# KTH-RPL/cloth-splatting

Hardware: AMD Instinct MI355X
Metric: rasterizer fwd+bwd rendered Mpix/s (scene_1, 800x800) (higher is better)
Workload: dtype f32

## Files before the change

cloth-splatting_amd/csrc/csplat_raster.hip:

```cpp
#include "csplat_common.h"

#include <atomic>
#include <cstring>
#include <chrono>
#include <mutex>
#include <type_traits>

namespace {

constexpr float NEAR_Z = 0.2f;
constexpr int RASTER_MAX_VIEWS = 8;

__device__ constexpr float SH_C0 = 0.28209479177387814f;
__device__ constexpr float SH_C1 = 0.4886025119029199f;
__device__ constexpr float SH_C2[5] = {1.0925484305920792f, -1.0925484305920792f, 0.31539156525252005f,
                                       -1.0925484305920792f, 0.5462742152960396f};
__device__ constexpr float SH_C3[7] = {-0.5900435899266435f, 2.890611442640554f, -0.4570457994644658f,
                                       0.3731763325901154f, -0.4570457994644658f, 1.445305721320277f,
                                       -0.5900435899266435f};

struct Geom {
    float *depth;
    float2 *xy;
    float4 *conic_opacity;
// ... 406 lines not shown
    extern __shared__ uint32_t s_hist[];
    for (int t = threadIdx.x; t < tiles; t += BUCKET_G) s_hist[t] = 0u;
    __syncthreads();
    const int i = blockIdx.x * BUCKET_G + threadIdx.x;
    if (i < P) {
        const int rad = radii[i];
        if (rad > 0) {
            const float2 p = xy[i];
            int minx, miny, maxx, maxy;
            tile_rect(p.x, p.y, rad, cam, minx, miny, maxx, maxy);
            for (int y = miny; y < maxy; y++)
                for (int x = minx; x < maxx; x++) atomicAdd(&s_hist[y * cam.gx + x], 1u);
        }
    }
    __syncthreads();
    uint32_t *row = table + (size_t)blockIdx.x * tiles;
    for (int t = threadIdx.x; t < tiles; t += BUCKET_G) row[t] = s_hist[t];
}
__global__ __launch_bounds__(BUCKET_G) void k_tile_count(int P, int tiles, const float2 *__restrict__ xy,
                                                          const int32_t *__restrict__ radii, Cam cam,
                                                          uint32_t *__restrict__ table) {
    tile_count_body(P, tiles, xy, radii, cam, table);
}
__global__ __launch_bounds__(BUCKET_G) void k_tile_count_views(int P, int tiles, K1Table tab) {
    const K1View &w = tab.v[blockIdx.y];
    tile_count_body(P, tiles, w.g.xy, w.radii, w.cam, w.table);
}

__device__ __forceinline__ void tile_colscan_body(int tiles, int nb, uint32_t *__restrict__ table, uint32_t *__restrict__ cnt) {
    const int t = blockIdx.x * 256 + threadIdx.x;
    if (t >= tiles) return;
    uint32_t run = 0;
    int b = 0;
    for (; b + 8 <= nb; b += 8) {
        uint32_t v[8];
#pragma unroll
        for (int u = 0; u < 8; u++) v[u] = table[(size_t)(b + u) * tiles + t];
#pragma unroll
        for (int u = 0; u < 8; u++) { table[(size_t)(b + u) * tiles + t] = run; run += v[u]; }
    }
    for (; b < nb; b++) { const uint32_t v = table[(size_t)b * tiles + t]; table[(size_t)b * tiles + t] = run; run += v; }
    cnt[t] = run;
}
__global__ __launch_bounds__(256) void k_tile_colscan(int tiles, int nb, uint32_t *__restrict__ table, uint32_t *__restrict__ cnt) {
    tile_colscan_body(tiles, nb, table, cnt);
}
__global__ __launch_bounds__(256) void k_tile_colscan_views(int tiles, int nb, K1Table tab) {
    uint32_t *table = tab.v[blockIdx.y].table;
    tile_colscan_body(tiles, nb, table, table + (size_t)nb * tiles);
}

constexpr int INFO_BUSY = 64;
constexpr int LPT_BINS = 512;
__device__ __forceinline__ void tile_scan_body(int tiles, const uint32_t *__restrict__ cnt, int2 *__restrict__ ranges,
                                               uint32_t *__restrict__ info, volatile uint32_t *mailbox, uint32_t tag) {
    __shared__ unsigned long long s_w[17];
    __shared__ uint32_t s_max[16];
    const int lane = threadIdx.x & 63, w = threadIdx.x >> 6;
    unsigned long long carry = 0ull;
    uint32_t mx = 0;
    uint32_t *busy = info + INFO_BUSY;
    for (int base = 0; base < tiles; base += 1024) {
        const int t = base + threadIdx.x;
        const uint32_t c = t < tiles ? cnt[t] : 0u;
        mx = max(mx, c);
        const unsigned long long v0 = (unsigned long long)c | ((unsigned long long)(c ? 1u : 0u) << 32);
        unsigned long long inc = v0;
#pragma unroll
        for (int d = 1; d < 64; d <<= 1) { const unsigned long long o = __shfl_up(inc, d, 64); if (lane >= d) inc += o; }
        if (lane == 63) s_w[w] = inc;
        __syncthreads();
        if (w == 0) {
            unsigned long long v = lane < 16 ? s_w[lane] : 0ull, vi = v;
#pragma unroll
            for (int d = 1; d < 16; d <<= 1) { const unsigned long long o = __shfl_up(vi, d, 64); if (lane >= d) vi += o; }
            if (lane < 16) s_w[lane] = vi - v;
            if (lane == 15) s_w[16] = vi;
        }
        __syncthreads();
        const unsigned long long exl = carry + s_w[w] + inc - v0;
        const uint32_t ex = (uint32_t)exl;
        if (t < tiles) {
            ranges[t] = c ? make_int2((int)ex, (int)(ex + c)) : make_int2(0, 0);
            if (c) busy[1 + (uint32_t)(exl >> 32)] = (uint32_t)t;
            else busy[tiles + 4 + tiles - 1 - (t - (int)(uint32_t)(exl >> 32))] = (uint32_t)t;
        }
        carry += s_w[16];
        __syncthreads();
    }
    {
        __shared__ uint32_t s_bin[LPT_BINS + 1];
        const uint32_t nbusy = (uint32_t)(carry >> 32);
        uint32_t *lpt = busy + tiles + 4;
        for (int i = threadIdx.x; i <= LPT_BINS; i += 1024) s_bin[i] = 0u;
        __syncthreads();
        for (uint32_t i = threadIdx.x; i < nbusy; i += 1024) {
            const uint32_t c = cnt[busy[1 + i]];
            atomicAdd(&s_bin[LPT_BINS - 1 - min(c >> 4, (uint32_t)(LPT_BINS - 1))], 1u);
        }
        __syncthreads();
        if (w == 0) {
            uint32_t v[LPT_BINS / 64], run = 0;
#pragma unroll
            for (int k = 0; k < LPT_BINS / 64; k++) { v[k] = s_bin[lane * (LPT_BINS / 64) + k]; run += v[k]; }
            uint32_t inc = run;
#pragma unroll
            for (int d = 1; d < 64; d <<= 1) { const uint32_t o = (uint32_t)__shfl_up((int)inc, d, 64); if (lane >= d) inc += o; }
            uint32_t base = inc - run;
#pragma unroll
            for (int k = 0; k < LPT_BINS / 64; k++) { s_bin[lane * (LPT_BINS / 64) + k] = base; base += v[k]; }
        }
        __syncthreads();
        for (uint32_t i = threadIdx.x; i < nbusy; i += 1024) {
            const uint32_t t = busy[1 + i], c = cnt[t];
            lpt[atomicAdd(&s_bin[LPT_BINS - 1 - min(c >> 4, (uint32_t)(LPT_BINS - 1))], 1u)] = t;
        }
    }
#pragma unroll
    for (int d = 32; d > 0; d >>= 1) mx = max(mx, (uint32_t)__shfl_xor((int)mx, d, 64));
    if (lane == 0) s_max[w] = mx;
    __syncthreads();
    if (threadIdx.x == 0) {
        uint32_t m = 0;
        for (int k = 0; k < 16; k++) m = max(m, s_max[k]);
        info[0] = (uint32_t)carry;
        info[1] = m;
        info[2] = (uint32_t)(carry >> 32);
        busy[0] = (uint32_t)(carry >> 32);
        if (mailbox) {
            mailbox[0] = (uint32_t)carry;
            mailbox[1] = m;
            mailbox[3] = (uint32_t)(carry >> 32);
            __threadfence_system();
            mailbox[2] = tag;
        }
    }
}
__global__ __launch_bounds__(1024) void k_tile_scan(int tiles, const uint32_t *__restrict__ cnt, int2 *__restrict__ ranges,
                                                     uint32_t *__restrict__ info, volatile uint32_t *mailbox, uint32_t tag) {
    tile_scan_body(tiles, cnt, ranges, info, mailbox, tag);
}
__global__ __launch_bounds__(1024) void k_tile_scan_views(int tiles, int nb, K1Table tab) {
    const K1View &w = tab.v[blockIdx.x];
    tile_scan_body(tiles, w.table + (size_t)nb * tiles, w.ranges, w.info, w.mailbox, w.tag);
}

__device__ __forceinline__ void emit_bucket_body(int P, int tiles, const float2 *__restrict__ xy,
                                                 const float *__restrict__ depth, const int32_t *__restrict__ radii,
                                                 const Cam &cam, const uint32_t *__restrict__ table,
                                                 const int2 *__restrict__ ranges, uint64_t *__restrict__ comp) {
    extern __shared__ uint32_t s_base[];
    const uint32_t *row = table + (size_t)blockIdx.x * tiles;
    for (int t = threadIdx.x; t < tiles; t += BUCKET_G) s_base[t] = (uint32_t)ranges[t].x + row[t];
    __syncthreads();
    const int i = blockIdx.x * BUCKET_G + threadIdx.x;
    if (i >= P) return;
    const int rad = radii[i];
    if (rad <= 0) return;
    const float2 p = xy[i];
    int minx, miny, maxx, maxy;
    tile_rect(p.x, p.y, rad, cam, minx, miny, maxx, maxy);
    const uint64_t v = ((uint64_t)__float_as_uint(depth[i]) << 32) | (uint32_t)i;
    for (int y = miny; y < maxy; y++)
        for (int x = minx; x < maxx; x++) comp[atomicAdd(&s_base[y * cam.gx + x], 1u)] = v;
}
__global__ __launch_bounds__(BUCKET_G) void k_emit_bucket(int P, int tiles, const float2 *__restrict__ xy,
                                                           const float *__restrict__ depth, const int32_t *__restrict__ radii,
                                                           Cam cam, const uint32_t *__restrict__ table,
                                                           const int2 *__restrict__ ranges, uint64_t *__restrict__ comp) {
    emit_bucket_body(P, tiles, xy, depth, radii, cam, table, ranges, comp);
}

struct P2View {
    Geom g;
    Cam cam;
    const int32_t *radii;
    const uint32_t *table;
    int2 *ranges;
    uint64_t *keys_u, *keys_sorted;
    uint32_t *ids_sorted;
    int *seg_offset, *slot_tile;
    float4 *ckpt;
    uint16_t *mask16;
    unsigned long long *bbits;
    unsigned long long *bmask;
    float4 *recA, *recB;
    float2 *recC;
    const float *bg;
    float *final_T;
    uint32_t *n_contrib;
    float *out_color, *out_depth;
    uint32_t R;
    const uint32_t *info;
    uint32_t Lcap;
    uint32_t Bcap;
    int spec;
};
struct P2Table { P2View v[RASTER_MAX_VIEWS]; uint32_t *valid; int nviews; };
__device__ __forceinline__ bool p2_live(const P2View &w) { return !w.spec || (w.info[0] - 1u < w.R && w.info[1] <= w.Lcap && w.info[2] <= w.Bcap); }
__device__ __forceinline__ void seg_plan_body(int tiles, const int2 *__restrict__ ranges, int *__restrict__ seg_offset,
                                              int *__restrict__ slot_tile);
__global__ __launch_bounds__(BUCKET_G) void k_emit_bucket_views(int P, int tiles, P2Table tab) {
    const P2View &w = tab.v[blockIdx.y];
    if (!p2_live(w)) return;
    if (blockIdx.x == gridDim.x - 1) { seg_plan_body(tiles, w.ranges, w.seg_offset, w.slot_tile); return; }
    emit_bucket_body(P, tiles, w.g.xy, w.g.depth, w.radii, w.cam, w.table, w.ranges, w.keys_u);
}

constexpr int TSORT_THREADS = 1024;
constexpr int TSORT_WAVES = TSORT_THREADS / 64;
constexpr int TSORT_ITEMS = BUCKET_CAP / TSORT_THREADS;
constexpr int TSORT_NB = 4 * TSORT_THREADS;
constexpr int TSORT_GRID = 512;
constexpr int TSORT_LONG = 64;
constexpr int TSORT_WORDS = TSORT_NB + 4 + 256 + 8 + 2 + 2 + TSORT_WAVES + 2;
__host__ __device__ inline size_t tsort_lds_bytes(int longest) {
    const int items = (longest > 0 ? longest : 1) + TSORT_THREADS - 1;
    return (size_t)(items / TSORT_THREADS) * TSORT_THREADS * 8 + (size_t)TSORT_WORDS * 4;
}

__device__ __forceinline__ void tile_sort_body(const int2 *__restrict__ ranges, const uint64_t *__restrict__ comp,
                                               uint64_t *__restrict__ keys_sorted,
                                               uint32_t *__restrict__ ids_sorted, int mode, int tile) {
    extern __shared__ uint64_t s_key[];
    const int2 r = ranges[tile];
    const int n = r.y - r.x;
    if (n <= 0) return;
    const int skip_byte3 = mode & 1;
    const int items = (n + TSORT_THREADS - 1) / TSORT_THREADS;
    uint32_t *s_cnt = reinterpret_cast<uint32_t *>(s_key + (size_t)items * TSORT_THREADS);
    uint32_t *s_dig = s_cnt + TSORT_NB + 4;
    const int lane = threadIdx.x & 63, w = threadIdx.x >> 6;
    const int wbase = w * items * 64;
    const uint64_t lt = (1ull << lane) - 1ull;
    uint64_t key[TSORT_ITEMS];
    uint32_t rank[TSORT_ITEMS];
#pragma unroll
    for (int i = 0; i < TSORT_ITEMS; i++) {
        const int idx = wbase + i * 64 + lane;
        key[i] = (i < items && idx < n) ? comp[r.x + idx] : ~0ull;
    }
    uint32_t *s_diff = s_dig + 264;
    uint32_t *s_mm = s_diff + 2;
    uint32_t *s_wtot = s_mm + 2;
    const uint64_t hi = (uint64_t)(uint32_t)tile << 32;
    if (!(mode & 2)) {
        uint32_t dmin = ~0u, dmax = 0u;
#pragma unroll
        for (int i = 0; i < TSORT_ITEMS; i++) {
            const int idx = wbase + i * 64 + lane;
            if (i < items && idx < n) { const uint32_t d = (uint32_t)(key[i] >> 32); dmin = min(dmin, d); dmax = max(dmax, d); }
        }
#pragma unroll
        for (int o = 32; o > 0; o >>= 1) {
            dmin = min(dmin, (uint32_t)__shfl_xor((int)dmin, o, 64));
            dmax = max(dmax, (uint32_t)__shfl_xor((int)dmax, o, 64));
        }
        if (threadIdx.x == 0) { s_mm[0] = ~0u; s_mm[1] = 0u; }
        reinterpret_cast<uint4 *>(s_cnt)[threadIdx.x] = make_uint4(0u, 0u, 0u, 0u);
        __syncthreads();
        if (lane == 0) { atomicMin(&s_mm[0], dmin); atomicMax(&s_mm[1], dmax); }
        __syncthreads();
        dmin = s_mm[0]; dmax = s_mm[1];
        if (dmax != dmin) {
            const float scale = (float)TSORT_NB / ((float)(dmax - dmin) + 1.0f);
            uint32_t bs[TSORT_ITEMS];
#pragma unroll
            for (int i = 0; i < TSORT_ITEMS; i++) {
                const int idx = wbase + i * 64 + lane;
                if (i < items && idx < n) {
                    const uint32_t b = min((uint32_t)(TSORT_NB - 1), (uint32_t)((float)((uint32_t)(key[i] >> 32) - dmin) * scale));
                    bs[i] = (b << 16) | atomicAdd(&s_cnt[b], 1u);
                }
            }
            __syncthreads();
            const uint4 c = reinterpret_cast<const uint4 *>(s_cnt)[threadIdx.x];
            const uint32_t tot = c.x + c.y + c.z + c.w;
            uint32_t inc = tot;
#pragma unroll
            for (int dd = 1; dd < 64; dd <<= 1) { const uint32_t o = __shfl_up(inc, dd, 64); if (lane >= dd) inc += o; }
            if (lane == 63) s_wtot[w] = inc;
            __syncthreads();
            uint32_t ex = inc - tot;
            for (int k = 0; k < w; k++) ex += s_wtot[k];
            reinterpret_cast<uint4 *>(s_cnt)[threadIdx.x] = make_uint4(ex, ex + c.x, ex + c.x + c.y, ex + c.x + c.y + c.z);
            if (threadIdx.x == 0) s_cnt[TSORT_NB] = (uint32_t)n;
            __syncthreads();
#pragma unroll
            for (int i = 0; i < TSORT_ITEMS; i++) {
                const int idx = wbase + i * 64 + lane;
                if (i < items && idx < n) s_key[s_cnt[bs[i] >> 16] + (bs[i] & 0xFFFFu)] = key[i];
            }
            __syncthreads();
            const int limit = (mode & 4) ? 1 : TSORT_LONG;
            bool long_run = false;
            uint32_t dst[TSORT_ITEMS];
#pragma unroll
            for (int i = 0; i < TSORT_ITEMS; i++) {
                const int idx = wbase + i * 64 + lane;
                if (i < items && idx < n) {
                    const uint32_t b = bs[i] >> 16;
                    const uint32_t lo = s_cnt[b], cb = s_cnt[b + 1] - lo;
                    uint32_t rk = 0;
                    if (cb > (uint32_t)limit) long_run = true;
                    else
                        for (uint32_t j = 0; j < cb; j++) rk += s_key[lo + j] < key[i] ? 1u : 0u;
                    dst[i] = lo + rk;
                }
            }
            if (!__syncthreads_or(long_run)) {
#pragma unroll
                for (int i = 0; i < TSORT_ITEMS; i++) {
                    const int idx = wbase + i * 64 + lane;
                    if (i < items && idx < n) s_key[dst[i]] = key[i];
                }
                __syncthreads();
#pragma unroll
                for (int i = 0; i < TSORT_ITEMS; i++) {
                    const int idx = wbase + i * 64 + lane;
                    if (i < items && idx < n) {
                        const uint64_t k = s_key[idx];
                        keys_sorted[r.x + idx] = hi | (k >> 32);
                        ids_sorted[r.x + idx] = (uint32_t)k;
                    }
                }
                return;
            }
        }
    }
    __syncthreads();
    if (threadIdx.x < 2) s_diff[threadIdx.x] = 0u;
    __syncthreads();
    {
        const uint64_t k0 = comp[r.x];
        uint64_t dv = 0ull;
#pragma unroll
        for (int i = 0; i < TSORT_ITEMS; i++) {
            const int idx = wbase + i * 64 + lane;
            if (i < items && idx < n) dv |= key[i] ^ k0;
        }
        uint32_t lo = (uint32_t)dv, hi32 = (uint32_t)(dv >> 32);
#pragma unroll
        for (int o = 32; o > 0; o >>= 1) { lo |= (uint32_t)__shfl_xor((int)lo, o, 64); hi32 |= (uint32_t)__shfl_xor((int)hi32, o, 64); }
        if (lane == 0) { atomicOr(&s_diff[0], lo); atomicOr(&s_diff[1], hi32); }
    }
    __syncthreads();
    const uint64_t diffbits = (uint64_t)s_diff[0] | ((uint64_t)s_diff[1] << 32);
    auto pass = [&](int shift) {
        for (int t = threadIdx.x; t < TSORT_WAVES * 256; t += TSORT_THREADS) s_cnt[t] = 0u;
        __syncthreads();
#pragma unroll
        for (int i = 0; i < TSORT_ITEMS; i++) {
            if (i < items) {
                const int idx = wbase + i * 64 + lane;
                const bool valid = idx < n;
                const uint32_t d = (uint32_t)(key[i] >> shift) & 0xFF;
                unsigned long long peers = __builtin_amdgcn_ballot_w64(valid);
#pragma unroll
                for (int b = 0; b < 8; b++) {
                    const unsigned long long mb = __builtin_amdgcn_ballot_w64(valid && ((d >> b) & 1));
                    peers &= ((d >> b) & 1) ? mb : ~mb;
                }
                const uint32_t prev = s_cnt[w * 256 + d];
                rank[i] = prev + (uint32_t)__popcll(peers & lt);
                __builtin_amdgcn_wave_barrier();
                if (valid && (peers & lt) == 0ull) s_cnt[w * 256 + d] = prev + (uint32_t)__popcll(peers);
                __builtin_amdgcn_wave_barrier();
            }
        }
        __syncthreads();
        uint32_t c[TSORT_WAVES];
        uint32_t tot = 0;
        if (threadIdx.x < 256) {
#pragma unroll
            for (int k = 0; k < TSORT_WAVES; k++) { c[k] = s_cnt[k * 256 + threadIdx.x]; tot += c[k]; }
            uint32_t inc = tot;
#pragma unroll
            for (int dd = 1; dd < 64; dd <<= 1) { const uint32_t o = __shfl_up(inc, dd, 64); if (lane >= dd) inc += o; }
            if (lane == 63) s_dig[256 + w] = inc;
            s_dig[threadIdx.x] = inc - tot;
        }
        __syncthreads();
        if (threadIdx.x < 256) {
            uint32_t run = s_dig[threadIdx.x];
            for (int k = 0; k < w; k++) run += s_dig[256 + k];
#pragma unroll
            for (int k = 0; k < TSORT_WAVES; k++) { s_cnt[k * 256 + threadIdx.x] = run; run += c[k]; }
        }
        __syncthreads();
#pragma unroll
        for (int i = 0; i < TSORT_ITEMS; i++) {
            if (i < items) {
                const int idx = wbase + i * 64 + lane;
                if (idx < n) {
                    const uint32_t d = (uint32_t)(key[i] >> shift) & 0xFF;
                    s_key[s_cnt[w * 256 + d] + rank[i]] = key[i];
                }
            }
        }
        __syncthreads();
#pragma unroll
        for (int i = 0; i < TSORT_ITEMS; i++) {
            const int idx = wbase + i * 64 + lane;
            if (i < items && idx < n) key[i] = s_key[idx];
        }
        __syncthreads();
    };
    auto varies = [&](int byte) { return ((diffbits >> (byte * 8)) & 0xFFull) != 0ull && !(byte == 3 && skip_byte3); };
    constexpr int TIE_RUN = 8;
    bool full = (diffbits >> 32) == 0ull;
    if (!full) {
        for (int byte = 4; byte < 8; byte++)
            if (varies(byte)) pass(byte * 8);
        bool long_run = false;
#pragma unroll
        for (int i = 0; i < TSORT_ITEMS; i++) {
            const int idx = wbase + i * 64 + lane;
            if (i < items && idx + 1 < n) {
                const uint32_t d = (uint32_t)(key[i] >> 32);
                const bool starts = (idx == 0 || (uint32_t)(s_key[idx - 1] >> 32) != d) && (uint32_t)(s_key[idx + 1] >> 32) == d;
                if (starts) {
                    int j = idx + 2;
                    while (j < n && j - idx <= TIE_RUN && (uint32_t)(s_key[j] >> 32) == d) j++;
                    if (j - idx > TIE_RUN) long_run = true;
                    else
                        for (int a2 = idx + 1; a2 < j; a2++) {
                            const uint64_t v = s_key[a2];
                            int b2 = a2 - 1;
                            while (b2 >= idx && s_key[b2] > v) { s_key[b2 + 1] = s_key[b2]; b2--; }
                            s_key[b2 + 1] = v;
                        }
                }
            }
        }
        full = __syncthreads_or(long_run);
        if (!full) {
#pragma unroll
            for (int i = 0; i < TSORT_ITEMS; i++) {
                const int idx = wbase + i * 64 + lane;
                if (i < items && idx < n) key[i] = s_key[idx];
            }
        }
    }
    if (full)
        for (int byte = 0; byte < 8; byte++)
            if (varies(byte)) pass(byte * 8);
#pragma unroll
    for (int i = 0; i < TSORT_ITEMS; i++) {
        const int idx = wbase + i * 64 + lane;
        if (i < items && idx < n) {
            keys_sorted[r.x + idx] = hi | (key[i] >> 32);
            ids_sorted[r.x + idx] = (uint32_t)key[i];
        }
    }
}
__global__ __launch_bounds__(TSORT_THREADS) void k_tile_sort(const int2 *__restrict__ ranges, const uint64_t *__restrict__ comp,
                                                              uint64_t *__restrict__ keys_sorted,
                                                              uint32_t *__restrict__ ids_sorted, const uint32_t *__restrict__ info, int mode) {
    const uint32_t *busy = info + INFO_BUSY;
    const int nbusy = (int)busy[0];
    for (int b = blockIdx.x; b < nbusy; b += gridDim.x) {
        tile_sort_body(ranges, comp, keys_sorted, ids_sorted, mode, (int)busy[1 + b]);
        __syncthreads();
    }
}
__global__ __launch_bounds__(TSORT_THREADS) void k_tile_sort_views(P2Table tab, int mode) {
    const P2View &w = tab.v[blockIdx.y];
    if (!p2_live(w)) return;
    const uint32_t *busy = w.info + INFO_BUSY;
    const int nbusy = (int)busy[0];
    for (int b = blockIdx.x; b < nbusy; b += gridDim.x) {
        tile_sort_body(w.ranges, w.keys_u, w.keys_sorted, w.ids_sorted, mode, (int)busy[1 + b]);
        __syncthreads();
    }
}

template <int CTRL, int RMASK>
__device__ __forceinline__ float dpp_mov(float v, float old) {
    return __int_as_float(__builtin_amdgcn_update_dpp(__float_as_int(old), __float_as_int(v), CTRL, RMASK, 0xF, false));
}
__device__ __forceinline__ float wave_min(float v) {
    v = fminf(v, dpp_mov<0xB1, 0xF>(v, v)); v = fminf(v, dpp_mov<0x4E, 0xF>(v, v));
    v = fminf(v, dpp_mov<0x141, 0xF>(v, v)); v = fminf(v, dpp_mov<0x140, 0xF>(v, v));
    const float r0 = __int_as_float(__builtin_amdgcn_readlane(__float_as_int(v), 0));
    const float r1 = __int_as_float(__builtin_amdgcn_readlane(__float_as_int(v), 16));
    const float r2 = __int_as_float(__builtin_amdgcn_readlane(__float_as_int(v), 32));
    const float r3 = __int_as_float(__builtin_amdgcn_readlane(__float_as_int(v), 48));
    return fminf(fminf(r0, r1), fminf(r2, r3));
}
__device__ __forceinline__ float wave_max(float v) { return -wave_min(-v); }

__device__ __forceinline__ bool box_hit(float2 c, float cut2, float4 co, float bx0, float bx1, float by0, float by1, bool exact) {
    const float lx = bx0 - c.x, hx = bx1 - c.x, ly = by0 - c.y, hy = by1 - c.y;
    const float ex = fmaxf(lx, fminf(0.f, hx)), ey = fmaxf(ly, fminf(0.f, hy));
    if (!(ex * ex + ey * ey <= cut2)) return false;
    if (!exact || cut2 > 1.0e30f) return true;
    const float A = co.x, B = co.y, C = co.z;
    float qmin = 0.f, sabs = 0.f;
    if (ex != 0.f || ey != 0.f) {
        float q1 = 3.0e38f, s1 = 0.f, q2 = 3.0e38f, s2 = 0.f;
        if (ex != 0.f) {
            const float dy = fminf(fmaxf(-B * ex * __builtin_amdgcn_rcpf(fmaxf(C, 1e-30f)), ly), hy);
            const float t0 = A * ex * ex, t1 = 2.f * B * ex * dy, t2 = C * dy * dy;
            q1 = t0 + t1 + t2; s1 = t0 + fabsf(t1) + t2;
        }
        if (ey != 0.f) {
            const float dx = fminf(fmaxf(-B * ey * __builtin_amdgcn_rcpf(fmaxf(A, 1e-30f)), lx), hx);
            const float t0 = C * ey * ey, t1 = 2.f * B * ey * dx, t2 = A * dx * dx;
            q2 = t0 + t1 + t2; s2 = t0 + fabsf(t1) + t2;
        }
        const bool first = q1 <= q2;
        qmin = first ? q1 : q2; sabs = first ? s1 : s2;
    }
    const float tau = 2.f * __logf(255.f * co.w);
    return qmin - 1e-5f * sabs <= tau * 1.001f + 1e-3f;
}

#ifndef CSPLAT_SEG
#define CSPLAT_SEG 256
#endif
constexpr int SEG = CSPLAT_SEG;

__device__ __forceinline__ void seg_plan_body(int tiles, const int2 *__restrict__ ranges, int *__restrict__ seg_offset,
                                              int *__restrict__ slot_tile) {
    __shared__ int s_w[17];
// ... 2309 lines not shown
        k_tile_scan_views<<<V, 1024, 0, join>>>(tiles, nb, tab);
        LAUNCH_CHECK();
    }
    return 0;
}

int csplat_forward_begin(void *stream, int P, int D, int M, const float *bg, int W, int H, const float *means3D,
                         const float *shs, const float *colors_precomp, const float *opacities, const float *scales,
                         float scale_modifier, const float *rotations, const float *cov3D_precomp, const float *view,
                         const float *proj, const float *campos, float tanfovx, float tanfovy, int prefiltered,
                         csplat_alloc_fn alloc, void *alloc_ctx, int32_t *radii, int *ticket_out) {
    CSPLAT_REQUIRE(!(prefiltered & CSPLAT_ANTIALIAS), "csplat_forward / csplat_forward_begin: CSPLAT_ANTIALIAS needs a csplat_view entry point "
                                                      "(csplat_forward_views*), whose backward knows the bit");
    if (int rc = begin_prepare(stream, P, D, M, bg, W, H, means3D, shs, colors_precomp, opacities, scales, scale_modifier, rotations,
                               cov3D_precomp, view, proj, campos, tanfovx, tanfovy, prefiltered, alloc, alloc_ctx, radii, ticket_out))
        return rc;
    const int rc = begin_launch(g_tickets[*ticket_out]);
    if (rc) {
        std::lock_guard<std::mutex> lk(g_ticket_mu);
        g_tickets[*ticket_out].used = false;
    }
    return rc;
}

static int finish_read(const FwdTicket &t, uint32_t host_info[3], hipStream_t launched_on = nullptr) {
    hipStream_t s = launched_on ? launched_on : t.s;
    host_info[0] = host_info[1] = host_info[2] = 0;
    if (t.can_bucket) {
        bool got = false;
        if (t.use_mail) {
            const auto t0 = std::chrono::steady_clock::now();
            unsigned spins = 0;
            while (!(got = (t.mb_host[2] == t.tag))) {
                if ((++spins & 0x3FFu) == 0 &&
                    std::chrono::duration<double>(std::chrono::steady_clock::now() - t0).count() > 2.0) break;
            }
            if (got) { host_info[0] = t.mb_host[0]; host_info[1] = t.mb_host[1]; host_info[2] = t.mb_host[3]; }
        }
        if (!got) {
            HIP_TRY(hipMemcpyAsync(host_info, t.info, 12, hipMemcpyDeviceToHost, s));
            HIP_TRY(hipStreamSynchronize(s));
        }
    } else if (t.P > 0) {
        ProfScope ps(PROF_K2, s);
        if (int rc = csplat_inclusive_scan_u32(s, t.g.tiles_touched, t.g.offsets, t.P, t.g.scan_tmp)) return rc;
        HIP_TRY(hipMemcpyAsync(host_info, t.g.offsets + (t.P - 1), 4, hipMemcpyDeviceToHost, s));
        HIP_TRY(hipStreamSynchronize(s));
        host_info[1] = 0xFFFFFFFFu;
        host_info[2] = 0xFFFFFFFFu;
    }
    CSPLAT_REQUIRE(host_info[0] <= 0x7FFFFFFFu, "csplat_forward: more than 2^31 - 1 tile instances (Gaussian x tile pairs) in one view");
    return 0;
}
static uint32_t tile_sort_cap() {
    static int s_lds_big = -1;
    if (s_lds_big < 0) {
        s_lds_big = hipFuncSetAttribute((const void *)k_tile_sort, hipFuncAttributeMaxDynamicSharedMemorySize, 96 * 1024) == hipSuccess &&
                    hipFuncSetAttribute((const void *)k_tile_sort_views, hipFuncAttributeMaxDynamicSharedMemorySize, 96 * 1024) == hipSuccess;
        (void)hipGetLastError();
    }
    return s_lds_big ? (uint32_t)BUCKET_CAP : 5120u;
}

struct SpecHist { int W = 0, H = 0, P = 0; uint32_t R = 0, longest = 0, busy = 0; };
constexpr int SPEC_RING = 8;
static SpecHist g_spec_ring[SPEC_RING];
static int g_spec_next = 0;
static std::mutex g_spec_mu;

struct PendingViews {
    bool used = false;
    const csplat_view *key = nullptr;
    int V = 0, tk[RASTER_MAX_VIEWS];
    uint32_t Rcap[RASTER_MAX_VIEWS], Lcap = 0, Bcap = 0;
};
constexpr int MAX_PENDING = 8;
static PendingViews g_pending[MAX_PENDING];
static std::mutex g_pending_mu;

static int p2_launch(int V, const int *tk, csplat_view *v, hipStream_t join, const uint32_t *Rcap, uint32_t Lcap, int spec, uint32_t Bcap,
                     uint32_t *valid = nullptr) {
    const FwdTicket &a = g_tickets[tk[0]];
    const int P = a.P, W = a.W, H = a.H, tiles = a.tiles, nb = a.nb;
    {
        P2Table tab;
        tab.valid = valid; tab.nviews = V;
        uint32_t maxR = 0;
        for (int i = 0; i < V; i++) {
            const FwdTicket &t = g_tickets[tk[i]];
            const uint32_t R = Rcap[i];
            maxR = R > maxR ? R : maxR;
            void *bbase = t.alloc(t.alloc_ctx, CSPLAT_CHUNK_BINNING, csplat_binning_bytes(R, W, H));
            void *tbase = t.alloc(t.alloc_ctx, CSPLAT_CHUNK_TEMP, csplat_temp_bytes(P, R, W, H));
            CSPLAT_REQUIRE(bbase && tbase, "allocator returned NULL");
            const BinView b = binning_view(bbase, R, tiles);
            P2View &k = tab.v[i];
            k.g = t.g; k.cam = t.cam; k.radii = t.radii; k.table = t.table; k.ranges = t.ranges;
            k.keys_u = temp_view(tbase, R).keys_u;
            k.keys_sorted = b.keys_sorted; k.ids_sorted = b.ids_sorted; k.seg_offset = b.seg_offset; k.slot_tile = b.slot_tile;
            k.ckpt = b.ckpt; k.mask16 = b.mask16; k.bbits = b.bbits; k.bmask = b.bmask; k.recA = b.recA; k.recB = b.recB; k.recC = b.recC;
            k.bg = t.bg; k.final_T = t.final_T; k.n_contrib = t.n_contrib; k.out_color = v[i].out_color; k.out_depth = v[i].out_depth;
            k.R = R; k.info = t.info; k.Lcap = Lcap; k.Bcap = Bcap; k.spec = spec;
            v[i].layout_rendered = (int)R; v[i].geom = t.gbase; v[i].binning = bbase; v[i].image = t.ibase;
        }
        {
            ProfScope ps(PROF_K3, join);
            k_emit_bucket_views<<<dim3(nb + 1, V), BUCKET_G, (size_t)tiles * 4, join>>>(P, tiles, tab);
            LAUNCH_CHECK();
        }
        {
            const size_t lds = tsort_lds_bytes((int)Lcap);
            ProfScope ps(PROF_K4, join);
            k_tile_sort_views<<<dim3(tiles < TSORT_GRID ? tiles : TSORT_GRID, V), TSORT_THREADS, lds, join>>>(tab, tsort_mode(P));
            LAUNCH_CHECK();
        }
        {
            ProfScope ps(PROF_K5, join);
            const int exact = (g_debug_flags & (1u | 16u | 32u)) ? 0 : 1, nbm = cdiv((int64_t)maxR + 1, 256);
            if (V == 1 || V == 2 || V == 4 || V == 8)
                k_block_masks_views<<<dim3((unsigned)(((int64_t)nbm * V + 7) / 8 * 8)), 256, 0, join>>>(tab, exact, V);
            else
                k_block_masks_views<<<dim3(nbm, V), 256, 0, join>>>(tab, exact, 0);
            LAUNCH_CHECK();
        }
        {
            ProfScope ps(PROF_K6, join);
            const int total = cdiv(tiles, 8) * 128, bg_ = cdiv((int)Bcap, 8) * 128, busy_grid = bg_ < total ? bg_ : total;
            if (!(g_debug_flags & 32768u))
                k_composite_fwd_views<false><<<dim3(busy_grid + K6_EXTRA, V), 64, 0, join>>>(tiles, W, H, tab, busy_grid);
            else
                k_composite_fwd_views<true><<<dim3(busy_grid + K6_EXTRA, V), 64, 0, join>>>(tiles, W, H, tab, busy_grid);
            LAUNCH_CHECK();
        }
        return 0;
    }
}

static int finish_views_batched(int V, const int *tk, csplat_view *v, hipStream_t join, bool *done, int mode = 0,
                                PendingViews *pend = nullptr, int *relaunched = nullptr) {
    *done = false;
    if (V < 1 || V > RASTER_MAX_VIEWS || (g_debug_flags & 512u)) return 0;
    const FwdTicket &a = g_tickets[tk[0]];
    for (int i = 0; i < V; i++) {
        const FwdTicket &t = g_tickets[tk[i]];
        if (!t.can_bucket || t.P != a.P || t.W != a.W || t.H != a.H || t.P <= 0) return 0;
    }
    const int P = a.P, W = a.W, H = a.H, tiles = a.tiles;
    const uint32_t cap = tile_sort_cap();
    uint32_t info[RASTER_MAX_VIEWS][3];
    bool have_info = false;
    auto read_counts = [&]() -> int {
        for (int i = 0; i < V && !have_info; i++)
            if (int rc = finish_read(g_tickets[tk[i]], info[i], join)) return rc;
        have_info = true;
        return 0;
    };
    auto launch = [&](const uint32_t *Rcap, uint32_t Lcap, int spec, uint32_t Bcap) -> int { return p2_launch(V, tk, v, join, Rcap, Lcap, spec, Bcap); };
    auto remember = [&]() {
        std::lock_guard<std::mutex> lk(g_spec_mu);
        SpecHist &e = g_spec_ring[g_spec_next];
        g_spec_next = (g_spec_next + 1) % SPEC_RING;
        e.W = W; e.H = H; e.P = P; e.R = 0; e.longest = 0; e.busy = 0;
        for (int i = 0; i < V; i++) {
            e.R = info[i][0] > e.R ? info[i][0] : e.R;
            e.longest = info[i][1] > e.longest ? info[i][1] : e.longest;
            e.busy = info[i][2] > e.busy ? info[i][2] : e.busy;
// ... 55 lines not shown
        longest = info[i][1] > longest ? info[i][1] : longest;
        busiest = info[i][2] > busiest ? info[i][2] : busiest;
        Rex[i] = info[i][0];
    }
    remember();
    if (int rc = launch(Rex, longest, 0, busiest)) return rc;
    if (relaunched) *relaunched = 1;
    for (int i = 0; i < V; i++) { v[i].num_rendered = (int)info[i][0]; v[i].busy_tiles = (int)info[i][2]; }
    release();
    *done = true;
    return 0;
}

int csplat_forward_finish(int ticket, float *out_color, float *out_depth, int *num_rendered, void **geom_out,
                          void **binning_out, void **image_out) {
    CSPLAT_REQUIRE(ticket >= 0 && ticket < MAX_TICKETS && g_tickets[ticket].used, "csplat_forward_finish: unknown ticket");
    const FwdTicket t = g_tickets[ticket];
    {
        std::lock_guard<std::mutex> lk(g_ticket_mu);
        g_tickets[ticket].used = false;
    }
    hipStream_t s = t.s;
    const int P = t.P, W = t.W, H = t.H, tiles = t.tiles, nb = t.nb;
    const bool can_bucket = t.can_bucket;
    const Cam cam = t.cam;
    const Geom g = t.g;
    void *gbase = t.gbase, *ibase = t.ibase;
    int2 *ranges = t.ranges;
    uint32_t *n_contrib = t.n_contrib, *table = t.table;
    float *final_T = t.final_T;
    const float *bg = t.bg;
    int32_t *radii = t.radii;
    csplat_alloc_fn alloc = t.alloc;
    void *alloc_ctx = t.alloc_ctx;
    uint32_t host_info[3] = {0, 0, 0};
    if (int rc = finish_read(t, host_info)) return rc;
    const uint32_t R = host_info[0];
    const uint32_t cap = tile_sort_cap();
    const bool bucketed = can_bucket && host_info[1] <= cap;
    *num_rendered = (int)R;
    void *bbase = alloc(alloc_ctx, CSPLAT_CHUNK_BINNING, csplat_binning_bytes(R, W, H));
    CSPLAT_REQUIRE(bbase, "allocator returned NULL");
    const BinView b = binning_view(bbase, R, tiles);
    if (R > 0) {
        void *tbase = alloc(alloc_ctx, CSPLAT_CHUNK_TEMP, csplat_temp_bytes(P, R, W, H));
        CSPLAT_REQUIRE(tbase, "allocator returned NULL");
        const TempView tmp = temp_view(tbase, R);
        if (bucketed) {
            {
                ProfScope ps(PROF_K3, s);
                k_emit_bucket<<<nb, BUCKET_G, (size_t)tiles * 4, s>>>(P, tiles, g.xy, g.depth, radii, cam, table, ranges, tmp.keys_u);
                LAUNCH_CHECK();
            }
            const size_t lds = tsort_lds_bytes((int)host_info[1]);
            ProfScope ps(PROF_K4, s);
            k_tile_sort<<<tiles < TSORT_GRID ? tiles : TSORT_GRID, TSORT_THREADS, lds, s>>>(ranges, tmp.keys_u, b.keys_sorted, b.ids_sorted, t.info, tsort_mode(P));
            LAUNCH_CHECK();
        } else {
            if (can_bucket) {
                ProfScope ps(PROF_K2, s);
                if (int rc = csplat_inclusive_scan_u32(s, g.tiles_touched, g.offsets, P, g.scan_tmp)) return rc;
            }
            {
                ProfScope ps(PROF_K3, s);
                k_emit_keys<<<cdiv(P, 256), 256, 0, s>>>(P, g.xy, g.depth, g.offsets, radii, cam, tmp.keys_u, tmp.ids_u);
                LAUNCH_CHECK();
            }
            const int end_bit = 32 + higher_msb((uint32_t)tiles);
            {
                ProfScope ps(PROF_K4, s);
                if (int rc = csplat_sort_pairs(s, tmp.keys_u, tmp.ids_u, b.keys_sorted, b.ids_sorted, tmp.keys_t, tmp.ids_t, R, end_bit, tmp.sort_tmp))
                    return rc;
            }
            {
                ProfScope ps(PROF_K5, s);
                HIP_TRY(hipMemsetAsync(ranges, 0, (size_t)tiles * 8, s));
                k_tile_ranges<<<cdiv(R, 256), 256, 0, s>>>(R, b.keys_sorted, ranges);
                LAUNCH_CHECK();
            }
        }
    }
    {
        ProfScope ps(PROF_K5, s);
        k_seg_plan<<<1, 1024, 0, s>>>(tiles, ranges, b.seg_offset, b.slot_tile);
        LAUNCH_CHECK();
    }
    {
        ProfScope ps(PROF_K5, s);
        k_block_masks<<<cdiv((int64_t)R + 1, 256), 256, 0, s>>>((int64_t)R, cam.gx, b.keys_sorted, b.ids_sorted, g.pack, b.mask16, b.recA, b.recB,
                                                                 b.recC, (g_debug_flags & (1u | 16u | 32u)) ? 0 : 1, b.bmask);
        LAUNCH_CHECK();
    }
    {
        ProfScope ps(PROF_K6, s);
        if (g_debug_flags & 32768u)
            k_composite_fwd<true><<<cdiv(tiles, 8) * 128, 64, 0, s>>>(tiles, W, H, cam.gx, ranges, b.mask16, b.recA, b.recB, b.recC, R, bg, b.seg_offset,
                                                                      b.ckpt, final_T, n_contrib, out_color, out_depth, b.bbits, b.bmask);
        else
            k_composite_fwd<false><<<cdiv(tiles, 8) * 128, 64, 0, s>>>(tiles, W, H, cam.gx, ranges, b.mask16, b.recA, b.recB, b.recC, R, bg, b.seg_offset,
                                                                       b.ckpt, final_T, n_contrib, out_color, out_depth, b.bbits, b.bmask);
        LAUNCH_CHECK();
    }
    *geom_out = gbase; *binning_out = bbase; *image_out = ibase;
    return 0;
}

int csplat_forward(void *stream, int P, int D, int M, const float *bg, int W, int H, const float *means3D,
                   const float *shs, const float *colors_precomp, const float *opacities, const float *scales,
                   float scale_modifier, const float *rotations, const float *cov3D_precomp, const float *view,
// ... 822 lines not shown
```

Baseline: 4645.

## Template tile sort on item count, occupancy hints, LPT tile order, blocked tile scan

The per-tile sort kernel is templated on the number of items per thread, chosen on the host from the longest tile, so short tiles need fewer registers. A denser launch-bounds variant is picked when many tiles are busy. The sort now walks tiles in the LPT (largest-first) order, and multi-view blocks are interleaved across views. The tile scan kernel is restructured to a single blocked pass that builds the LPT histogram inline instead of looping and rereading counts. This adds several kernel instantiations and a device-attribute query, and the tighter launch bounds risk register spills.

```diff
diff --git a/cloth-splatting_amd/csrc/csplat_raster.hip b/cloth-splatting_amd/csrc/csplat_raster.hip
--- a/cloth-splatting_amd/csrc/csplat_raster.hip
+++ b/cloth-splatting_amd/csrc/csplat_raster.hip
@@ -482,69 +482,73 @@
 
 constexpr int INFO_BUSY = 64;
 constexpr int LPT_BINS = 512;
+constexpr int TSCAN_ITEMS = BUCKET_TILES / 1024;
 __device__ __forceinline__ void tile_scan_body(int tiles, const uint32_t *__restrict__ cnt, int2 *__restrict__ ranges,
                                                uint32_t *__restrict__ info, volatile uint32_t *mailbox, uint32_t tag) {
     __shared__ unsigned long long s_w[17];
     __shared__ uint32_t s_max[16];
+    __shared__ uint32_t s_bin[LPT_BINS + 1];
     const int lane = threadIdx.x & 63, w = threadIdx.x >> 6;
-    unsigned long long carry = 0ull;
+    uint32_t *busy = info + INFO_BUSY;
+    uint32_t *lpt = busy + tiles + 4;
+    const int per = (tiles + 1023) / 1024, t0 = threadIdx.x * per;
+    uint32_t c[TSCAN_ITEMS];
+#pragma unroll
+    for (int k = 0; k < TSCAN_ITEMS; k++) c[k] = (k < per && t0 + k < tiles) ? cnt[t0 + k] : 0u;
+    for (int i = threadIdx.x; i <= LPT_BINS; i += 1024) s_bin[i] = 0u;
     uint32_t mx = 0;
-    uint32_t *busy = info + INFO_BUSY;
-    for (int base = 0; base < tiles; base += 1024) {
-        const int t = base + threadIdx.x;
-        const uint32_t c = t < tiles ? cnt[t] : 0u;
-        mx = max(mx, c);
-        const unsigned long long v0 = (unsigned long long)c | ((unsigned long long)(c ? 1u : 0u) << 32);
-        unsigned long long inc = v0;
-#pragma unroll
-        for (int d = 1; d < 64; d <<= 1) { const unsigned long long o = __shfl_up(inc, d, 64); if (lane >= d) inc += o; }
-        if (lane == 63) s_w[w] = inc;
-        __syncthreads();
-        if (w == 0) {
-            unsigned long long v = lane < 16 ? s_w[lane] : 0ull, vi = v;
-#pragma unroll
-            for (int d = 1; d < 16; d <<= 1) { const unsigned long long o = __shfl_up(vi, d, 64); if (lane >= d) vi += o; }
-            if (lane < 16) s_w[lane] = vi - v;
-            if (lane == 15) s_w[16] = vi;
-        }
-        __syncthreads();
-        const unsigned long long exl = carry + s_w[w] + inc - v0;
-        const uint32_t ex = (uint32_t)exl;
-        if (t < tiles) {
-            ranges[t] = c ? make_int2((int)ex, (int)(ex + c)) : make_int2(0, 0);
-            if (c) busy[1 + (uint32_t)(exl >> 32)] = (uint32_t)t;
-            else busy[tiles + 4 + tiles - 1 - (t - (int)(uint32_t)(exl >> 32))] = (uint32_t)t;
-        }
-        carry += s_w[16];
-        __syncthreads();
-    }
+    unsigned long long v0 = 0ull;
+#pragma unroll
+    for (int k = 0; k < TSCAN_ITEMS; k++) { mx = max(mx, c[k]); v0 += (unsigned long long)c[k] | ((unsigned long long)(c[k] ? 1u : 0u) << 32); }
+    unsigned long long inc = v0;
+#pragma unroll
+    for (int d = 1; d < 64; d <<= 1) { const unsigned long long o = __shfl_up(inc, d, 64); if (lane >= d) inc += o; }
+    if (lane == 63) s_w[w] = inc;
+    __syncthreads();
+    if (w == 0) {
+        unsigned long long v = lane < 16 ? s_w[lane] : 0ull, vi = v;
+#pragma unroll
+        for (int d = 1; d < 16; d <<= 1) { const unsigned long long o = __shfl_up(vi, d, 64); if (lane >= d) vi += o; }
+        if (lane < 16) s_w[lane] = vi - v;
+        if (lane == 15) s_w[16] = vi;
+    }
+    __syncthreads();
+    const unsigned long long carry = s_w[16];
     {
-        __shared__ uint32_t s_bin[LPT_BINS + 1];
-        const uint32_t nbusy = (uint32_t)(carry >> 32);
-        uint32_t *lpt = busy + tiles + 4;
-        for (int i = threadIdx.x; i <= LPT_BINS; i += 1024) s_bin[i] = 0u;
-        __syncthreads();
-        for (uint32_t i = threadIdx.x; i < nbusy; i += 1024) {
-            const uint32_t c = cnt[busy[1 + i]];
-            atomicAdd(&s_bin[LPT_BINS - 1 - min(c >> 4, (uint32_t)(LPT_BINS - 1))], 1u);
-        }
-        __syncthreads();
+        unsigned long long exl = s_w[w] + inc - v0;
+#pragma unroll
+        for (int k = 0; k < TSCAN_ITEMS; k++) {
+            const int t = t0 + k;
+            if (k < per && t < tiles) {
+                const uint32_t ex = (uint32_t)exl, nz = (uint32_t)(exl >> 32);
+                ranges[t] = c[k] ? make_int2((int)ex, (int)(ex + c[k])) : make_int2(0, 0);
+                if (c[k]) {
+                    busy[1 + nz] = (uint32_t)t;
+                    atomicAdd(&s_bin[LPT_BINS - 1 - min(c[k] >> 4, (uint32_t)(LPT_BINS - 1))], 1u);
+                } else {
+                    lpt[tiles - 1 - (t - (int)nz)] = (uint32_t)t;
+                }
+                exl += (unsigned long long)c[k] | ((unsigned long long)(c[k] ? 1u : 0u) << 32);
+            }
+        }
+    }
+    __syncthreads();
+    {
         if (w == 0) {
             uint32_t v[LPT_BINS / 64], run = 0;
 #pragma unroll
             for (int k = 0; k < LPT_BINS / 64; k++) { v[k] = s_bin[lane * (LPT_BINS / 64) + k]; run += v[k]; }
-            uint32_t inc = run;
-#pragma unroll
-            for (int d = 1; d < 64; d <<= 1) { const uint32_t o = (uint32_t)__shfl_up((int)inc, d, 64); if (lane >= d) inc += o; }
-            uint32_t base = inc - run;
+            uint32_t binc = run;
+#pragma unroll
+            for (int d = 1; d < 64; d <<= 1) { const uint32_t o = (uint32_t)__shfl_up((int)binc, d, 64); if (lane >= d) binc += o; }
+            uint32_t base = binc - run;
 #pragma unroll
             for (int k = 0; k < LPT_BINS / 64; k++) { s_bin[lane * (LPT_BINS / 64) + k] = base; base += v[k]; }
         }
         __syncthreads();
-        for (uint32_t i = threadIdx.x; i < nbusy; i += 1024) {
-            const uint32_t t = busy[1 + i], c = cnt[t];
-            lpt[atomicAdd(&s_bin[LPT_BINS - 1 - min(c >> 4, (uint32_t)(LPT_BINS - 1))], 1u)] = t;
-        }
+#pragma unroll
+        for (int k = 0; k < TSCAN_ITEMS; k++)
+            if (c[k]) lpt[atomicAdd(&s_bin[LPT_BINS - 1 - min(c[k] >> 4, (uint32_t)(LPT_BINS - 1))], 1u)] = (uint32_t)(t0 + k);
     }
 #pragma unroll
     for (int d = 32; d > 0; d >>= 1) mx = max(mx, (uint32_t)__shfl_xor((int)mx, d, 64));
@@ -639,7 +643,6 @@
 
 constexpr int TSORT_THREADS = 1024;
 constexpr int TSORT_WAVES = TSORT_THREADS / 64;
-constexpr int TSORT_ITEMS = BUCKET_CAP / TSORT_THREADS;
 constexpr int TSORT_NB = 4 * TSORT_THREADS;
 constexpr int TSORT_GRID = 512;
 constexpr int TSORT_LONG = 64;
@@ -649,6 +652,7 @@
     return (size_t)(items / TSORT_THREADS) * TSORT_THREADS * 8 + (size_t)TSORT_WORDS * 4;
 }
 
+template <int ITEMS>
 __device__ __forceinline__ void tile_sort_body(const int2 *__restrict__ ranges, const uint64_t *__restrict__ comp,
                                                uint64_t *__restrict__ keys_sorted,
                                                uint32_t *__restrict__ ids_sorted, int mode, int tile) {
@@ -660,13 +664,14 @@
     const int items = (n + TSORT_THREADS - 1) / TSORT_THREADS;
     uint32_t *s_cnt = reinterpret_cast<uint32_t *>(s_key + (size_t)items * TSORT_THREADS);
     uint32_t *s_dig = s_cnt + TSORT_NB + 4;
-    const int lane = threadIdx.x & 63, w = threadIdx.x >> 6;
+    int lane = threadIdx.x & 63, w = threadIdx.x >> 6;
+    asm volatile("" : "+v"(lane), "+v"(w));
     const int wbase = w * items * 64;
     const uint64_t lt = (1ull << lane) - 1ull;
-    uint64_t key[TSORT_ITEMS];
-    uint32_t rank[TSORT_ITEMS];
-#pragma unroll
-    for (int i = 0; i < TSORT_ITEMS; i++) {
+    uint64_t key[ITEMS];
+    uint32_t rank[ITEMS];
+#pragma unroll
+    for (int i = 0; i < ITEMS; i++) {
         const int idx = wbase + i * 64 + lane;
         key[i] = (i < items && idx < n) ? comp[r.x + idx] : ~0ull;
     }
@@ -677,7 +682,7 @@
     if (!(mode & 2)) {
         uint32_t dmin = ~0u, dmax = 0u;
 #pragma unroll
-        for (int i = 0; i < TSORT_ITEMS; i++) {
+        for (int i = 0; i < ITEMS; i++) {
             const int idx = wbase + i * 64 + lane;
             if (i < items && idx < n) { const uint32_t d = (uint32_t)(key[i] >> 32); dmin = min(dmin, d); dmax = max(dmax, d); }
         }
@@ -694,9 +699,9 @@
         dmin = s_mm[0]; dmax = s_mm[1];
         if (dmax != dmin) {
             const float scale = (float)TSORT_NB / ((float)(dmax - dmin) + 1.0f);
-            uint32_t bs[TSORT_ITEMS];
-#pragma unroll
-            for (int i = 0; i < TSORT_ITEMS; i++) {
+            uint32_t bs[ITEMS];
+#pragma unroll
+            for (int i = 0; i < ITEMS; i++) {
                 const int idx = wbase + i * 64 + lane;
                 if (i < items && idx < n) {
                     const uint32_t b = min((uint32_t)(TSORT_NB - 1), (uint32_t)((float)((uint32_t)(key[i] >> 32) - dmin) * scale));
@@ -717,16 +722,16 @@
             if (threadIdx.x == 0) s_cnt[TSORT_NB] = (uint32_t)n;
             __syncthreads();
 #pragma unroll
-            for (int i = 0; i < TSORT_ITEMS; i++) {
+            for (int i = 0; i < ITEMS; i++) {
                 const int idx = wbase + i * 64 + lane;
                 if (i < items && idx < n) s_key[s_cnt[bs[i] >> 16] + (bs[i] & 0xFFFFu)] = key[i];
             }
             __syncthreads();
             const int limit = (mode & 4) ? 1 : TSORT_LONG;
             bool long_run = false;
-            uint32_t dst[TSORT_ITEMS];
-#pragma unroll
-            for (int i = 0; i < TSORT_ITEMS; i++) {
+            uint32_t dst[ITEMS];
+#pragma unroll
+            for (int i = 0; i < ITEMS; i++) {
                 const int idx = wbase + i * 64 + lane;
                 if (i < items && idx < n) {
                     const uint32_t b = bs[i] >> 16;
@@ -734,19 +739,20 @@
                     uint32_t rk = 0;
                     if (cb > (uint32_t)limit) long_run = true;
                     else
+#pragma unroll 1
                         for (uint32_t j = 0; j < cb; j++) rk += s_key[lo + j] < key[i] ? 1u : 0u;
                     dst[i] = lo + rk;
                 }
             }
             if (!__syncthreads_or(long_run)) {
 #pragma unroll
-                for (int i = 0; i < TSORT_ITEMS; i++) {
+                for (int i = 0; i < ITEMS; i++) {
                     const int idx = wbase + i * 64 + lane;
                     if (i < items && idx < n) s_key[dst[i]] = key[i];
                 }
                 __syncthreads();
 #pragma unroll
-                for (int i = 0; i < TSORT_ITEMS; i++) {
+                for (int i = 0; i < ITEMS; i++) {
                     const int idx = wbase + i * 64 + lane;
                     if (i < items && idx < n) {
                         const uint64_t k = s_key[idx];
@@ -765,7 +771,7 @@
         const uint64_t k0 = comp[r.x];
         uint64_t dv = 0ull;
 #pragma unroll
-        for (int i = 0; i < TSORT_ITEMS; i++) {
+        for (int i = 0; i < ITEMS; i++) {
             const int idx = wbase + i * 64 + lane;
             if (i < items && idx < n) dv |= key[i] ^ k0;
         }
@@ -780,7 +786,7 @@
         for (int t = threadIdx.x; t < TSORT_WAVES * 256; t += TSORT_THREADS) s_cnt[t] = 0u;
         __syncthreads();
 #pragma unroll
-        for (int i = 0; i < TSORT_ITEMS; i++) {
+        for (int i = 0; i < ITEMS; i++) {
             if (i < items) {
                 const int idx = wbase + i * 64 + lane;
                 const bool valid = idx < n;
@@ -799,11 +805,10 @@
             }
         }
         __syncthreads();
-        uint32_t c[TSORT_WAVES];
         uint32_t tot = 0;
         if (threadIdx.x < 256) {
 #pragma unroll
-            for (int k = 0; k < TSORT_WAVES; k++) { c[k] = s_cnt[k * 256 + threadIdx.x]; tot += c[k]; }
+            for (int k = 0; k < TSORT_WAVES; k++) tot += s_cnt[k * 256 + threadIdx.x];
             uint32_t inc = tot;
 #pragma unroll
             for (int dd = 1; dd < 64; dd <<= 1) { const uint32_t o = __shfl_up(inc, dd, 64); if (lane >= dd) inc += o; }
@@ -815,11 +820,11 @@
             uint32_t run = s_dig[threadIdx.x];
             for (int k = 0; k < w; k++) run += s_dig[256 + k];
 #pragma unroll
-            for (int k = 0; k < TSORT_WAVES; k++) { s_cnt[k * 256 + threadIdx.x] = run; run += c[k]; }
+            for (int k = 0; k < TSORT_WAVES; k++) { const uint32_t ck = s_cnt[k * 256 + threadIdx.x]; s_cnt[k * 256 + threadIdx.x] = run; run += ck; }
         }
         __syncthreads();
 #pragma unroll
-        for (int i = 0; i < TSORT_ITEMS; i++) {
+        for (int i = 0; i < ITEMS; i++) {
             if (i < items) {
                 const int idx = wbase + i * 64 + lane;
                 if (idx < n) {
@@ -830,7 +835,7 @@
         }
         __syncthreads();
 #pragma unroll
-        for (int i = 0; i < TSORT_ITEMS; i++) {
+        for (int i = 0; i < ITEMS; i++) {
             const int idx = wbase + i * 64 + lane;
             if (i < items && idx < n) key[i] = s_key[idx];
         }
@@ -844,7 +849,7 @@
             if (varies(byte)) pass(byte * 8);
         bool long_run = false;
 #pragma unroll
-        for (int i = 0; i < TSORT_ITEMS; i++) {
+        for (int i = 0; i < ITEMS; i++) {
             const int idx = wbase + i * 64 + lane;
             if (i < items && idx + 1 < n) {
                 const uint32_t d = (uint32_t)(key[i] >> 32);
@@ -866,7 +871,7 @@
         full = __syncthreads_or(long_run);
         if (!full) {
 #pragma unroll
-            for (int i = 0; i < TSORT_ITEMS; i++) {
+            for (int i = 0; i < ITEMS; i++) {
                 const int idx = wbase + i * 64 + lane;
                 if (i < items && idx < n) key[i] = s_key[idx];
             }
@@ -876,7 +881,7 @@
         for (int byte = 0; byte < 8; byte++)
             if (varies(byte)) pass(byte * 8);
 #pragma unroll
-    for (int i = 0; i < TSORT_ITEMS; i++) {
+    for (int i = 0; i < ITEMS; i++) {
         const int idx = wbase + i * 64 + lane;
         if (i < items && idx < n) {
             keys_sorted[r.x + idx] = hi | (key[i] >> 32);
@@ -884,23 +889,26 @@
         }
     }
 }
-__global__ __launch_bounds__(TSORT_THREADS) void k_tile_sort(const int2 *__restrict__ ranges, const uint64_t *__restrict__ comp,
+template <int ITEMS, bool DENSE>
+__global__ __launch_bounds__(TSORT_THREADS, DENSE ? 8 : 4) void k_tile_sort(const int2 *__restrict__ ranges, const uint64_t *__restrict__ comp,
                                                               uint64_t *__restrict__ keys_sorted,
-                                                              uint32_t *__restrict__ ids_sorted, const uint32_t *__restrict__ info, int mode) {
-    const uint32_t *busy = info + INFO_BUSY;
+                                                              uint32_t *__restrict__ ids_sorted, const uint32_t *__restrict__ info, int tiles, int mode) {
+    const uint32_t *busy = info + INFO_BUSY, *lpt = busy + tiles + 4;
     const int nbusy = (int)busy[0];
     for (int b = blockIdx.x; b < nbusy; b += gridDim.x) {
-        tile_sort_body(ranges, comp, keys_sorted, ids_sorted, mode, (int)busy[1 + b]);
+        tile_sort_body<ITEMS>(ranges, comp, keys_sorted, ids_sorted, mode, (int)lpt[b]);
         __syncthreads();
     }
 }
-__global__ __launch_bounds__(TSORT_THREADS) void k_tile_sort_views(P2Table tab, int mode) {
-    const P2View &w = tab.v[blockIdx.y];
+template <int ITEMS, bool DENSE>
+__global__ __launch_bounds__(TSORT_THREADS, DENSE ? 8 : 4) void k_tile_sort_views(P2Table tab, int tiles, int mode) {
+    const int lin = blockIdx.y * gridDim.x + blockIdx.x, nv = gridDim.y;
+    const P2View &w = tab.v[lin % nv];
     if (!p2_live(w)) return;
-    const uint32_t *busy = w.info + INFO_BUSY;
+    const uint32_t *busy = w.info + INFO_BUSY, *lpt = busy + tiles + 4;
     const int nbusy = (int)busy[0];
-    for (int b = blockIdx.x; b < nbusy; b += gridDim.x) {
-        tile_sort_body(w.ranges, w.keys_u, w.keys_sorted, w.ids_sorted, mode, (int)busy[1 + b]);
+    for (int b = lin / nv; b < nbusy; b += gridDim.x) {
+        tile_sort_body<ITEMS>(w.ranges, w.keys_u, w.keys_sorted, w.ids_sorted, mode, (int)lpt[b]);
         __syncthreads();
     }
 }
@@ -3316,14 +3324,63 @@
     CSPLAT_REQUIRE(host_info[0] <= 0x7FFFFFFFu, "csplat_forward: more than 2^31 - 1 tile instances (Gaussian x tile pairs) in one view");
     return 0;
 }
+#define TSORT_FOR_ITEMS(X) X(2) X(4) X(6) X(8)
+static int tsort_items(uint32_t longest) {
+    const uint32_t items = (longest + TSORT_THREADS - 1) / TSORT_THREADS;
+    return items <= 2 ? 2 : items <= 4 ? 4 : items <= 6 ? 6 : 8;
+}
+static bool tsort_dense(int items, uint64_t busy) {
+    static int s_cus = 0;
+    if (s_cus <= 0) {
+        int dev = 0;
+        if (hipGetDevice(&dev) != hipSuccess || hipDeviceGetAttribute(&s_cus, hipDeviceAttributeMultiprocessorCount, dev) != hipSuccess || s_cus <= 0)
+            s_cus = 256;
+        (void)hipGetLastError();
+    }
+    return items <= 6 && 2 * busy > 5 * (uint64_t)s_cus;
+}
 static uint32_t tile_sort_cap() {
     static int s_lds_big = -1;
     if (s_lds_big < 0) {
-        s_lds_big = hipFuncSetAttribute((const void *)k_tile_sort, hipFuncAttributeMaxDynamicSharedMemorySize, 96 * 1024) == hipSuccess &&
-                    hipFuncSetAttribute((const void *)k_tile_sort_views, hipFuncAttributeMaxDynamicSharedMemorySize, 96 * 1024) == hipSuccess;
+        bool ok = true;
+#define X(I) ok = ok && hipFuncSetAttribute((const void *)k_tile_sort<I, false>, hipFuncAttributeMaxDynamicSharedMemorySize, 96 * 1024) == hipSuccess && \
+                  hipFuncSetAttribute((const void *)k_tile_sort<I, I <= 6>, hipFuncAttributeMaxDynamicSharedMemorySize, 96 * 1024) == hipSuccess &&  \
+                  hipFuncSetAttribute((const void *)k_tile_sort_views<I, false>, hipFuncAttributeMaxDynamicSharedMemorySize, 96 * 1024) == hipSuccess && \
+                  hipFuncSetAttribute((const void *)k_tile_sort_views<I, I <= 6>, hipFuncAttributeMaxDynamicSharedMemorySize, 96 * 1024) == hipSuccess;
+        TSORT_FOR_ITEMS(X)
+#undef X
+        s_lds_big = ok;
         (void)hipGetLastError();
     }
     return s_lds_big ? (uint32_t)BUCKET_CAP : 5120u;
+}
+static void tile_sort_launch(hipStream_t s, int tiles, uint32_t longest, uint32_t busy, const int2 *ranges, const uint64_t *comp,
+                             uint64_t *keys_sorted, uint32_t *ids_sorted, const uint32_t *info, int mode) {
+    const size_t lds = tsort_lds_bytes((int)longest);
+    const int grid = tiles < TSORT_GRID ? tiles : TSORT_GRID, items = tsort_items(longest);
+    const bool dense = tsort_dense(items, busy);
+    switch (items) {
+#define X(I) case I:                                                                                                                        \
+        if (dense) k_tile_sort<I, I <= 6><<<grid, TSORT_THREADS, lds, s>>>(ranges, comp, keys_sorted, ids_sorted, info, tiles, mode);       \
+        else k_tile_sort<I, false><<<grid, TSORT_THREADS, lds, s>>>(ranges, comp, keys_sorted, ids_sorted, info, tiles, mode);              \
+        break;
+        TSORT_FOR_ITEMS(X)
+#undef X
+    }
+}
+static void tile_sort_views_launch(hipStream_t s, int tiles, int V, uint32_t Lcap, uint32_t Bcap, const P2Table &tab, int mode) {
+    const size_t lds = tsort_lds_bytes((int)Lcap);
+    const dim3 grid(tiles < TSORT_GRID ? tiles : TSORT_GRID, V);
+    const int items = tsort_items(Lcap);
+    const bool dense = tsort_dense(items, (uint64_t)V * (Bcap < (uint32_t)tiles ? Bcap : (uint32_t)tiles));
+    switch (items) {
+#define X(I) case I:                                                                                           \
+        if (dense) k_tile_sort_views<I, I <= 6><<<grid, TSORT_THREADS, lds, s>>>(tab, tiles, mode);            \
+        else k_tile_sort_views<I, false><<<grid, TSORT_THREADS, lds, s>>>(tab, tiles, mode);                   \
+        break;
+        TSORT_FOR_ITEMS(X)
+#undef X
+    }
 }
 
 struct SpecHist { int W = 0, H = 0, P = 0; uint32_t R = 0, longest = 0, busy = 0; };
@@ -3373,9 +3430,8 @@
             LAUNCH_CHECK();
         }
         {
-            const size_t lds = tsort_lds_bytes((int)Lcap);
             ProfScope ps(PROF_K4, join);
-            k_tile_sort_views<<<dim3(tiles < TSORT_GRID ? tiles : TSORT_GRID, V), TSORT_THREADS, lds, join>>>(tab, tsort_mode(P));
+            tile_sort_views_launch(join, tiles, V, Lcap, Bcap, tab, tsort_mode(P));
             LAUNCH_CHECK();
         }
         {
@@ -3537,9 +3593,8 @@
                 k_emit_bucket<<<nb, BUCKET_G, (size_t)tiles * 4, s>>>(P, tiles, g.xy, g.depth, radii, cam, table, ranges, tmp.keys_u);
                 LAUNCH_CHECK();
             }
-            const size_t lds = tsort_lds_bytes((int)host_info[1]);
             ProfScope ps(PROF_K4, s);
-            k_tile_sort<<<tiles < TSORT_GRID ? tiles : TSORT_GRID, TSORT_THREADS, lds, s>>>(ranges, tmp.keys_u, b.keys_sorted, b.ids_sorted, t.info, tsort_mode(P));
+            tile_sort_launch(s, tiles, host_info[1], host_info[2], ranges, tmp.keys_u, b.keys_sorted, b.ids_sorted, t.info, tsort_mode(P));
             LAUNCH_CHECK();
         } else {
             if (can_bucket) {
```

After: 4716 (median of 6 runs). 1.5% higher.
